# una-dinosauria/local-search-quantization

Measured on AMD Instinct MI355X. Metric: vectors encoded/sec (ICM, m=8 h=256), higher is better.
Workload: dtype f32

## Files before the change

local-search-quantization_amd/csrc/lsq_cost.h:

```cpp
#pragma once

#include "lsq_wave.h"

namespace {

__device__ inline bool perturb_record(uint64_t (&w)[2], int m, int npert, uint64_t seed, uint32_t it, uint64_t gi) {
    int need = npert < m ? npert : m;
    bool changed = false;
    for (int g = 0; 4 * g < m && need > 0; ++g) {
        const lsq_u32x4 sel = lsq_rng_block(seed, gi, it, LSQ_DOM_PERTURB, (uint32_t)g);
        const lsq_u32x4 vals = lsq_rng_block(seed, gi, it, LSQ_DOM_PERTURB, (uint32_t)(4 + g));
#pragma unroll
        for (int e = 0; e < 4; ++e) {
            const int pp = 4 * g + e;
            if (pp < m && need > 0 && lsq_mulhi32(sel.v[e], (uint32_t)(m - pp)) < (uint32_t)need) {
                const uint64_t val = lsq_mulhi32(vals.v[e], LSQ_H);
                const int sh = 8 * (pp & 7);
                changed |= (((w[pp >> 3] >> sh) & 0xffull) != val);
                w[pp >> 3] = (w[pp >> 3] & ~(0xffull << sh)) | (val << sh);
                --need;
            }
        }
    }
    return changed;
}

template <int CS>
__device__ inline void perturb_next_store(const lsq_perturb_next &pn, int64_t i, const uint32_t (&fin)[CS / 4], unsigned short vfin) {
    uint64_t w[2];
    w[0] = (uint64_t)fin[0] | ((uint64_t)fin[1] << 32);
    w[1] = (CS == 16) ? ((uint64_t)fin[CS / 4 - 2] | ((uint64_t)fin[CS / 4 - 1] << 32)) : 0ull;
#ifdef LSQ_TUNING
    if (pn.abl & 16) return;
    const bool changed = (pn.abl & 1) ? false : perturb_record(w, pn.m, pn.npert, pn.seed, pn.it, pn.goff + (uint64_t)i);
#else
    const bool changed = perturb_record(w, pn.m, pn.npert, pn.seed, pn.it, pn.goff + (uint64_t)i);
#endif
    uint64_t *q = reinterpret_cast<uint64_t *>(pn.dst + i * CS);
    q[0] = w[0];
    if (CS == 16) q[1] = w[1];
    if (pn.vdst) pn.vdst[i] = changed ? (unsigned short)0 : vfin;
}

template <int M, int MODE, int HASV, int NQ, bool EXTCNT = false>
__device__ inline void cost4_body(const float *__restrict__ X, const float *__restrict__ K,
                                  const uint8_t *rec, uint8_t *cur, float *__restrict__ prev,
                                  unsigned long long *__restrict__ counters, int64_t lo, int64_t n, int64_t w, int64_t nwaves, int d,
                                  const unsigned short *vnew, unsigned short *vcur, const lsq_perturb_next &pn, unsigned *cnt_ext = nullptr) {
    constexpr int CS = (M <= 8) ? 8 : 16;
    constexpr int RW = CS / 4;
    const int lane = threadIdx.x & 63;
    const int qtr = lane >> 4, lp = lane & 15;
    unsigned n_eq = 0, n_lt = 0;
    for (int64_t base = lo + w * 64; base < n; base += nwaves * 64) {
        const int64_t il = base + lane;
        const bool livel = il < n;
        const int64_t ic = livel ? il : n - 1;
        uint32_t rn[RW], cw[RW];
        float pl = 0.0f;
        unsigned short vc = 0, vn = 0;
        {
            const uint32_t *rp = reinterpret_cast<const uint32_t *>(rec + ic * CS), *cp = reinterpret_cast<const uint32_t *>(cur + ic * CS);
#pragma unroll
            for (int q = 0; q < RW; ++q) rn[q] = rp[q];
            if (MODE == 1) {
#pragma unroll
                for (int q = 0; q < RW; ++q) cw[q] = cp[q];
                pl = prev[ic];
            }
            if (HASV) vc = vcur[ic];
            if (HASV && MODE == 1) vn = vnew[ic];
        }
        bool same = (MODE == 1);
#pragma unroll
        for (int q = 0; q < RW; ++q) {
            if (MODE == 0) cw[q] = rn[q];
            same = same && (rn[q] == cw[q]);
        }
        const bool skip = livel && same && (pl == pl);
        const unsigned nskip = (unsigned)__popcll(__ballot(skip));
        if (lane == 0) n_eq += nskip;
        unsigned short vfin = vc;
        const bool merge_v = HASV && MODE == 1 && same && livel;
        if (merge_v) vfin = (unsigned short)(vfin | vn);
        uint64_t accepted = 0;
        float newp = 0.0f;
        uint64_t todo = __ballot(livel && !skip);
#ifdef LSQ_TUNING
        if (pn.abl & 8) todo = 0;
#endif
        int nsidx[4];
        bool nhv[4];
        auto pick = [&]() {
#pragma unroll
            for (int v = 0; v < 4; ++v) {
                nhv[v] = todo != 0;
                nsidx[v] = nhv[v] ? __builtin_ctzll(todo) : (v ? nsidx[0] : 0);
                if (nhv[v]) todo &= todo - 1;
            }
        };
        auto xrow = [&]() -> const float * {
            const int mys = qtr == 0 ? nsidx[0] : qtr == 1 ? nsidx[1] : qtr == 2 ? nsidx[2] : nsidx[3];
            return X + (base + mys) * (int64_t)d;
        };
        f32x4 xn[NQ];
        auto xload = [&](const float *x, int c0) {
#pragma unroll
            for (int g = 0; g < NQ; ++g) {
                const int t = c0 + 64 * g + 4 * lp;
                xn[g] = *reinterpret_cast<const f32x4 *>(x + (t < d ? t : 0));
            }
        };
        pick();
        const float *xnext = xrow();
        if (nhv[0]) xload(xnext, 0);
        while (nhv[0]) {
            int sidx[4];
            bool hv[4];
#pragma unroll
            for (int v = 0; v < 4; ++v) { sidx[v] = nsidx[v]; hv[v] = nhv[v]; }
            const float *x = xnext;
            pick();
            xnext = xrow();
            const bool live = qtr == 0 ? hv[0] : qtr == 1 ? hv[1] : qtr == 2 ? hv[2] : hv[3];
            uint32_t r[RW];
            float pc;
            {
                uint32_t rv4[4][RW];
                float pc4[4];
#pragma unroll
                for (int v = 0; v < 4; ++v) {
#pragma unroll
                    for (int q = 0; q < RW; ++q) rv4[v][q] = (uint32_t)__builtin_amdgcn_readlane((int)rn[q], sidx[v]);
                    pc4[v] = __int_as_float(__builtin_amdgcn_readlane(__float_as_int(pl), sidx[v]));
                }
#pragma unroll
                for (int q = 0; q < RW; ++q) r[q] = qtr == 0 ? rv4[0][q] : qtr == 1 ? rv4[1][q] : qtr == 2 ? rv4[2][q] : rv4[3][q];
                pc = qtr == 0 ? pc4[0] : qtr == 1 ? pc4[1] : qtr == 2 ? pc4[2] : pc4[3];
            }
            uint32_t kb[M];
#pragma unroll
            for (int k = 0; k < M; ++k) kb[k] = ((uint32_t)(k * LSQ_H) + ((r[k >> 2] >> (8 * (k & 3))) & 0xffu)) * (uint32_t)d;
            f32x4 p = (f32x4){0.f, 0.f, 0.f, 0.f};
            for (int c0 = 0; c0 < d; c0 += 64 * NQ) {
                f32x4 xv[NQ], kv[NQ][M];
                bool ok[NQ];
#pragma unroll
                for (int g = 0; g < NQ; ++g) {
                    const int t = c0 + 64 * g + 4 * lp;
                    ok[g] = t < d;
                    const uint32_t u = ok[g] ? (uint32_t)t : 0u;
                    xv[g] = xn[g];
#pragma unroll
                    for (int k = 0; k < M; ++k) kv[g][k] = *reinterpret_cast<const f32x4 *>(K + (size_t)(kb[k] + u));
                }
                if (c0 + 64 * NQ < d) xload(x, c0 + 64 * NQ);
                else xload(xnext, 0);
#pragma unroll
                for (int g = 0; g < NQ; ++g) {
                    f32x4 cb = (f32x4){0.f, 0.f, 0.f, 0.f};
#pragma unroll
                    for (int k = 0; k < M; ++k) cb = cb + kv[g][k];
                    const f32x4 rr = cb - xv[g];
                    const f32x4 sq = rr * rr;
                    p.x = p.x + (ok[g] ? sq.x : 0.0f);
                    p.y = p.y + (ok[g] ? sq.y : 0.0f);
                    p.z = p.z + (ok[g] ? sq.z : 0.0f);
                    p.w = p.w + (ok[g] ? sq.w : 0.0f);
                }
            }
            float v = (p.x + p.y) + (p.z + p.w);
            v = v + dpp_self<DPP_XOR1, 0xf>(v);
            v = v + dpp_self<DPP_XOR2, 0xf>(v);
            v = v + dpp_self<DPP_HALF_MIRROR, 0xf>(v);
            v = v + dpp_self<DPP_MIRROR, 0xf>(v);
            const float cost = v;
#pragma unroll
            for (int v2 = 0; v2 < 4; ++v2) {
                const float cv = __int_as_float(__builtin_amdgcn_readlane(__float_as_int(cost), 16 * v2));
                if (hv[v2] && lane == sidx[v2]) newp = cv;
            }
            if (MODE == 1) {
                const bool eq = live && (cost == pc), lt = live && (cost < pc);
                const uint64_t bl = __ballot(lt && lp == 0);
                const unsigned ne = (unsigned)__popcll(__ballot(eq && lp == 0)), nl = (unsigned)__popcll(bl);
#pragma unroll
                for (int v2 = 0; v2 < 4; ++v2)
                    if ((bl >> (16 * v2)) & 1ull) accepted |= 1ull << sidx[v2];
                if (lane == 0) { n_eq += ne; n_lt += nl; }
            }
        }
        const bool acc = (accepted >> lane) & 1ull;
        if (MODE == 0) {
            if (livel) prev[il] = newp;
        } else if (acc) {
            prev[il] = newp;
            uint32_t *qd = reinterpret_cast<uint32_t *>(cur + il * CS);
#pragma unroll
            for (int q = 0; q < RW; ++q) qd[q] = rn[q];
        }
        if (HASV && MODE == 1 && (acc || merge_v)) vcur[il] = acc ? vn : vfin;
        if (pn.on && livel) {
            uint32_t fin[RW];
#pragma unroll
            for (int q = 0; q < RW; ++q) fin[q] = acc ? rn[q] : cw[q];
            perturb_next_store<CS>(pn, il, fin, acc ? vn : vfin);
        }
    }
    if (MODE == 1) {
        unsigned *cnt_s;
        if constexpr (EXTCNT) cnt_s = cnt_ext;
        else { __shared__ unsigned cnt_own[2]; cnt_s = cnt_own; }
        if (threadIdx.x == 0) { cnt_s[0] = 0u; cnt_s[1] = 0u; }
        __syncthreads();
        if (lane == 0 && n_eq) atomicAdd(&cnt_s[0], n_eq);
        if (lane == 0 && n_lt) atomicAdd(&cnt_s[1], n_lt);
        __syncthreads();
        if (threadIdx.x == 0 && cnt_s[0]) atomicAdd(&counters[0], (unsigned long long)cnt_s[0]);
        if (threadIdx.x == 0 && cnt_s[1]) atomicAdd(&counters[1], (unsigned long long)cnt_s[1]);
    }
}


}
```

Baseline: 21.25 million.

## Software-pipeline codebook and X loads one chunk ahead across vector groups

Restructures the cost loop into a flat chunk stream covering both the dimension slices and successive groups of four vectors, so the codebook gathers (K rows) and X rows for the next chunk are issued while the current chunk's sums are computed. Before, only X was prefetched and the K gathers sat on the critical path of each chunk. The cost reduction and accept logic now run only when a vector's final chunk completes. In exchange, register pressure rises from the extra in-flight kv/xc buffers, which may lower occupancy, and a sched_barrier constrains how the compiler can order instructions.

```diff
diff --git a/local-search-quantization_amd/csrc/lsq_cost.h b/local-search-quantization_amd/csrc/lsq_cost.h
--- a/local-search-quantization_amd/csrc/lsq_cost.h
+++ b/local-search-quantization_amd/csrc/lsq_cost.h
@@ -41,6 +41,8 @@
     if (CS == 16) q[1] = w[1];
     if (pn.vdst) pn.vdst[i] = changed ? (unsigned short)0 : vfin;
 }
+
+template <bool B> struct lsq_bool { static constexpr bool value = B; };
 
 template <int M, int MODE, int HASV, int NQ, bool EXTCNT = false>
 __device__ inline void cost4_body(const float *__restrict__ X, const float *__restrict__ K,
@@ -89,106 +91,114 @@
 #ifdef LSQ_TUNING
         if (pn.abl & 8) todo = 0;
 #endif
-        int nsidx[4];
-        bool nhv[4];
-        auto pick = [&]() {
+        struct Chunk { int s[4]; bool h[4]; int c0; };
+        auto pick = [&](Chunk &c) {
+            c.c0 = 0;
 #pragma unroll
             for (int v = 0; v < 4; ++v) {
-                nhv[v] = todo != 0;
-                nsidx[v] = nhv[v] ? __builtin_ctzll(todo) : (v ? nsidx[0] : 0);
-                if (nhv[v]) todo &= todo - 1;
-            }
-        };
-        auto xrow = [&]() -> const float * {
-            const int mys = qtr == 0 ? nsidx[0] : qtr == 1 ? nsidx[1] : qtr == 2 ? nsidx[2] : nsidx[3];
-            return X + (base + mys) * (int64_t)d;
-        };
-        f32x4 xn[NQ];
-        auto xload = [&](const float *x, int c0) {
+                c.h[v] = todo != 0;
+                c.s[v] = c.h[v] ? __builtin_ctzll(todo) : (v ? c.s[0] : 0);
+                if (c.h[v]) todo &= todo - 1;
+            }
+        };
+        auto advance = [&](const Chunk &c) {
+            Chunk nc = c;
+            if (c.c0 + 64 * NQ < d) nc.c0 = c.c0 + 64 * NQ;
+            else pick(nc);
+            return nc;
+        };
+        auto mine = [&](const Chunk &c) { return qtr == 0 ? c.s[0] : qtr == 1 ? c.s[1] : qtr == 2 ? c.s[2] : c.s[3]; };
+        auto xload = [&](f32x4 &xd, const Chunk &c, int g) {
+            const int t = c.c0 + 64 * g + 4 * lp;
+            xd = *reinterpret_cast<const f32x4 *>(X + (base + mine(c)) * (int64_t)d + (t < d ? t : 0));
+        };
+        auto rsel = [&](const Chunk &c, uint32_t (&r)[RW]) {
+#pragma unroll
+            for (int q = 0; q < RW; ++q) {
+                uint32_t r4[4];
+#pragma unroll
+                for (int v = 0; v < 4; ++v) r4[v] = (uint32_t)__builtin_amdgcn_readlane((int)rn[q], c.s[v]);
+                r[q] = qtr == 0 ? r4[0] : qtr == 1 ? r4[1] : qtr == 2 ? r4[2] : r4[3];
+            }
+        };
+        f32x4 kv[NQ][M];
+        auto kload = [&](const Chunk &c, const uint32_t (&r)[RW], int g) {
+            const int t = c.c0 + 64 * g + 4 * lp;
+            const uint32_t u = t < d ? (uint32_t)t : 0u;
+#pragma unroll
+            for (int k = 0; k < M; ++k)
+                kv[g][k] = *reinterpret_cast<const f32x4 *>(K + (size_t)(((uint32_t)(k * LSQ_H) + ((r[k >> 2] >> (8 * (k & 3))) & 0xffu)) * (uint32_t)d + u));
+        };
+        Chunk ch;
+        pick(ch);
+        f32x4 xc[NQ];
+        Chunk nxt = ch;
+        if (ch.h[0]) {
+            uint32_t r[RW];
+            rsel(ch, r);
+#pragma unroll
+            for (int g = 0; g < NQ; ++g) { xload(xc[g], ch, g); kload(ch, r, g); }
+            nxt = advance(ch);
+        }
+        f32x4 p = (f32x4){0.f, 0.f, 0.f, 0.f};
+        auto chunk = [&](auto last) __attribute__((always_inline)) {
+            constexpr bool LAST = decltype(last)::value;
+            const Chunk nx2 = LAST ? nxt : advance(nxt);
+            uint32_t rnx[RW];
+            if (!LAST) rsel(nxt, rnx);
 #pragma unroll
             for (int g = 0; g < NQ; ++g) {
-                const int t = c0 + 64 * g + 4 * lp;
-                xn[g] = *reinterpret_cast<const f32x4 *>(x + (t < d ? t : 0));
-            }
-        };
-        pick();
-        const float *xnext = xrow();
-        if (nhv[0]) xload(xnext, 0);
-        while (nhv[0]) {
-            int sidx[4];
-            bool hv[4];
-#pragma unroll
-            for (int v = 0; v < 4; ++v) { sidx[v] = nsidx[v]; hv[v] = nhv[v]; }
-            const float *x = xnext;
-            pick();
-            xnext = xrow();
-            const bool live = qtr == 0 ? hv[0] : qtr == 1 ? hv[1] : qtr == 2 ? hv[2] : hv[3];
-            uint32_t r[RW];
-            float pc;
-            {
-                uint32_t rv4[4][RW];
-                float pc4[4];
-#pragma unroll
-                for (int v = 0; v < 4; ++v) {
-#pragma unroll
-                    for (int q = 0; q < RW; ++q) rv4[v][q] = (uint32_t)__builtin_amdgcn_readlane((int)rn[q], sidx[v]);
-                    pc4[v] = __int_as_float(__builtin_amdgcn_readlane(__float_as_int(pl), sidx[v]));
+                const bool ok = ch.c0 + 64 * g + 4 * lp < d;
+                f32x4 cb = (f32x4){0.f, 0.f, 0.f, 0.f};
+#pragma unroll
+                for (int k = 0; k < M; ++k) cb = cb + kv[g][k];
+                const f32x4 rr = cb - xc[g];
+                const f32x4 sq = rr * rr;
+                p.x = p.x + (ok ? sq.x : 0.0f);
+                p.y = p.y + (ok ? sq.y : 0.0f);
+                p.z = p.z + (ok ? sq.z : 0.0f);
+                p.w = p.w + (ok ? sq.w : 0.0f);
+                if (!LAST) {
+                    asm volatile("" : "+v"(p));
+                    __builtin_amdgcn_sched_barrier(0);
+                    kload(nxt, rnx, g);
+                    xload(xc[g], nxt, g);
                 }
-#pragma unroll
-                for (int q = 0; q < RW; ++q) r[q] = qtr == 0 ? rv4[0][q] : qtr == 1 ? rv4[1][q] : qtr == 2 ? rv4[2][q] : rv4[3][q];
-                pc = qtr == 0 ? pc4[0] : qtr == 1 ? pc4[1] : qtr == 2 ? pc4[2] : pc4[3];
-            }
-            uint32_t kb[M];
-#pragma unroll
-            for (int k = 0; k < M; ++k) kb[k] = ((uint32_t)(k * LSQ_H) + ((r[k >> 2] >> (8 * (k & 3))) & 0xffu)) * (uint32_t)d;
-            f32x4 p = (f32x4){0.f, 0.f, 0.f, 0.f};
-            for (int c0 = 0; c0 < d; c0 += 64 * NQ) {
-                f32x4 xv[NQ], kv[NQ][M];
-                bool ok[NQ];
-#pragma unroll
-                for (int g = 0; g < NQ; ++g) {
-                    const int t = c0 + 64 * g + 4 * lp;
-                    ok[g] = t < d;
-                    const uint32_t u = ok[g] ? (uint32_t)t : 0u;
-                    xv[g] = xn[g];
-#pragma unroll
-                    for (int k = 0; k < M; ++k) kv[g][k] = *reinterpret_cast<const f32x4 *>(K + (size_t)(kb[k] + u));
+            }
+            if (ch.c0 + 64 * NQ >= d) {
+                float v = (p.x + p.y) + (p.z + p.w);
+                v = v + dpp_self<DPP_XOR1, 0xf>(v);
+                v = v + dpp_self<DPP_XOR2, 0xf>(v);
+                v = v + dpp_self<DPP_HALF_MIRROR, 0xf>(v);
+                v = v + dpp_self<DPP_MIRROR, 0xf>(v);
+                const float cost = v;
+                p = (f32x4){0.f, 0.f, 0.f, 0.f};
+#pragma unroll
+                for (int v2 = 0; v2 < 4; ++v2) {
+                    const float cv = __int_as_float(__builtin_amdgcn_readlane(__float_as_int(cost), 16 * v2));
+                    if (ch.h[v2] && lane == ch.s[v2]) newp = cv;
                 }
-                if (c0 + 64 * NQ < d) xload(x, c0 + 64 * NQ);
-                else xload(xnext, 0);
-#pragma unroll
-                for (int g = 0; g < NQ; ++g) {
-                    f32x4 cb = (f32x4){0.f, 0.f, 0.f, 0.f};
-#pragma unroll
-                    for (int k = 0; k < M; ++k) cb = cb + kv[g][k];
-                    const f32x4 rr = cb - xv[g];
-                    const f32x4 sq = rr * rr;
-                    p.x = p.x + (ok[g] ? sq.x : 0.0f);
-                    p.y = p.y + (ok[g] ? sq.y : 0.0f);
-                    p.z = p.z + (ok[g] ? sq.z : 0.0f);
-                    p.w = p.w + (ok[g] ? sq.w : 0.0f);
+                if (MODE == 1) {
+                    const bool live = qtr == 0 ? ch.h[0] : qtr == 1 ? ch.h[1] : qtr == 2 ? ch.h[2] : ch.h[3];
+                    float pc4[4];
+#pragma unroll
+                    for (int v2 = 0; v2 < 4; ++v2) pc4[v2] = __int_as_float(__builtin_amdgcn_readlane(__float_as_int(pl), ch.s[v2]));
+                    const float pc = qtr == 0 ? pc4[0] : qtr == 1 ? pc4[1] : qtr == 2 ? pc4[2] : pc4[3];
+                    const bool eq = live && (cost == pc), lt = live && (cost < pc);
+                    const uint64_t bl = __ballot(lt && lp == 0);
+                    const unsigned ne = (unsigned)__popcll(__ballot(eq && lp == 0)), nl = (unsigned)__popcll(bl);
+#pragma unroll
+                    for (int v2 = 0; v2 < 4; ++v2)
+                        if ((bl >> (16 * v2)) & 1ull) accepted |= 1ull << ch.s[v2];
+                    if (lane == 0) { n_eq += ne; n_lt += nl; }
                 }
             }
-            float v = (p.x + p.y) + (p.z + p.w);
-            v = v + dpp_self<DPP_XOR1, 0xf>(v);
-            v = v + dpp_self<DPP_XOR2, 0xf>(v);
-            v = v + dpp_self<DPP_HALF_MIRROR, 0xf>(v);
-            v = v + dpp_self<DPP_MIRROR, 0xf>(v);
-            const float cost = v;
-#pragma unroll
-            for (int v2 = 0; v2 < 4; ++v2) {
-                const float cv = __int_as_float(__builtin_amdgcn_readlane(__float_as_int(cost), 16 * v2));
-                if (hv[v2] && lane == sidx[v2]) newp = cv;
-            }
-            if (MODE == 1) {
-                const bool eq = live && (cost == pc), lt = live && (cost < pc);
-                const uint64_t bl = __ballot(lt && lp == 0);
-                const unsigned ne = (unsigned)__popcll(__ballot(eq && lp == 0)), nl = (unsigned)__popcll(bl);
-#pragma unroll
-                for (int v2 = 0; v2 < 4; ++v2)
-                    if ((bl >> (16 * v2)) & 1ull) accepted |= 1ull << sidx[v2];
-                if (lane == 0) { n_eq += ne; n_lt += nl; }
-            }
+            ch = nxt;
+            nxt = nx2;
+        };
+        if (ch.h[0]) {
+            while (nxt.h[0]) chunk(lsq_bool<false>{});
+            chunk(lsq_bool<true>{});
         }
         const bool acc = (accepted >> lane) & 1ull;
         if (MODE == 0) {
```

Result: no change. 21.53 million (median of 6 runs) (+1.3%).
